# pdegenhardt/MinCostFlow

Hardware: AMD Instinct MI355X
Metric: pivots/sec + solve ms, NETGEN 100k-node/300k-arc; arc-scan GB/s vs HBM peak (higher is better)
Workload: dtype int64

## Files before the change

include/mcf_hip.h:

```cpp
#ifndef MCF_HIP_H
#define MCF_HIP_H

#include <stdint.h>

#ifdef __cplusplus
extern "C" {
#endif

#define MCF_API __attribute__((visibility("default")))

typedef enum mcf_status {
    MCF_OK = 0,
    MCF_ERR_INVALID = -1,
    MCF_ERR_NO_DEVICE = -2,
    MCF_ERR_HIP = -3,
    MCF_ERR_OVERFLOW = -4,
    MCF_ERR_TIMEOUT = -5,
    MCF_ERR_STATE = -6,
    MCF_ERR_IO = -7,
    MCF_ERR_COMM = -8
} mcf_status;

typedef enum mcf_pivot_rule { MCF_RULE_FIRST_ELIGIBLE = 0, MCF_RULE_BEST_ELIGIBLE = 1, MCF_RULE_BLOCK_SEARCH = 2,
                              MCF_RULE_CANDIDATE_LIST = 3, MCF_RULE_ALTERING_LIST = 4 } mcf_pivot_rule;
// ... 135 lines not shown
    int64_t scan_launches;
    int64_t update_launches;
    int64_t inline_updates;
    int64_t potential_nodes;
    int64_t arcs_scanned;
    int64_t timed_scans;
    double timed_scan_ns;
    double host_wait_ns;
    double host_launch_ns;
    int32_t scan_workgroups, scan_threads;
    int64_t bytes_per_scan;
    int64_t resident;
    int64_t resident_launches;
    int64_t resident_requests;
    double resident_scan_ns;
    double resident_kernel_ns;
    int64_t candidates;
    int64_t host_decided;
    int64_t arcs_checked;
    int32_t initial_block_size, current_block_size;
    int32_t comm_ranks;
    int32_t reserved;
    int64_t async_refreshes;
    int64_t scan_bytes_read;
    int64_t rc_layout;
    int64_t rc_recomputes;
    int64_t renumberings;
    int64_t heap_compactions;
    int64_t rc_reloads_in_grid;
    int64_t shift_grid;
    int64_t shift_lists;
    int64_t mirror_uploads;
    double phase_shift_ns, phase_values_ns, phase_scan_ns;
} mcf_engine_stats;
MCF_API int mcf_engine_get_stats(mcf_engine *e, mcf_engine_stats *out);
MCF_API int mcf_engine_reset_stats(mcf_engine *e);

MCF_API int mcf_engine_bench_scan(mcf_engine *e, int32_t reps, int32_t cold, int64_t flush_bytes,
                                  double *avg_ns, double *min_ns);

MCF_API int mcf_engine_bench_update(mcf_engine *e, int32_t count, int32_t reps, double *avg_ns, double *min_ns, int64_t *bytes);

MCF_API int mcf_engine_bench_search(mcf_engine *e, int32_t reps, double *avg_ns, double *min_ns);

MCF_API int mcf_comm_unique_id(uint8_t id_out[128]);
MCF_API int mcf_engine_comm_init(mcf_engine *e, const uint8_t id[128], int32_t rank, int32_t world);
MCF_API int mcf_engine_find_entering_sharded(mcf_engine *e, int32_t *found, int32_t *arc, int64_t *reduced_cost);

typedef struct mcf_exchange mcf_exchange;
MCF_API int mcf_exchange_open(mcf_exchange **out, const char *name, int32_t rank, int32_t world);
MCF_API void mcf_exchange_close(mcf_exchange *x);
MCF_API int mcf_exchange_all_gather(mcf_exchange *x, const mcf_candidate *mine, mcf_candidate *all );


typedef struct mcf_ns mcf_ns;

MCF_API int mcf_ns_create(mcf_ns **out, int32_t node_count, int32_t arc_count, const int32_t *source, const int32_t *target);
MCF_API void mcf_ns_destroy(mcf_ns *s);
MCF_API int mcf_ns_set_arc_bounds(mcf_ns *s, int32_t arc, int64_t lower, int64_t upper);
MCF_API int mcf_ns_set_arc_cost(mcf_ns *s, int32_t arc, int64_t cost);
MCF_API int mcf_ns_set_node_supply(mcf_ns *s, int32_t node, int64_t supply);
MCF_API int mcf_ns_set_problem(mcf_ns *s, const int64_t *lower, const int64_t *upper, const int64_t *cost, const int64_t *supply);
MCF_API int mcf_ns_set_supply_type(mcf_ns *s, int32_t type);
MCF_API int mcf_ns_set_pivot_rule(mcf_ns *s, int32_t rule);
MCF_API int mcf_ns_set_list_pivot_rule(mcf_ns *s, int32_t rule);
MCF_API int mcf_ns_enable_optimized_pivot(mcf_ns *s, int32_t enable);
// ... 442 lines not shown
```

mincostflow_amd/_lib.py:

```python
from __future__ import annotations

import ctypes as C
import importlib.util
import os
import re
import sys
import warnings

import numpy as np

_HERE = os.path.dirname(os.path.abspath(__file__))
LIB_PATH = os.path.join(_HERE, "libmcf_hip.so")

RULE_FIRST_ELIGIBLE, RULE_BEST_ELIGIBLE, RULE_BLOCK_SEARCH, RULE_CANDIDATE_LIST, RULE_ALTERING_LIST = 0, 1, 2, 3, 4
COLLECT_FIRST_N, COLLECT_BLOCKS = 0, 1
SEM_PLAIN, SEM_OPTIMIZED = 1, 2
VECTOR_DEFAULT, VECTOR_NONE = 0, -1
SUPPLY_GEQ, SUPPLY_LEQ = 0, 1
NOT_SOLVED, OPTIMAL, INFEASIBLE, UNBOUNDED, UNBALANCED = 0, 1, 2, 3, 4
STATE_UPPER, STATE_TREE, STATE_LOWER = -1, 0, 1
INF_CAP = np.iinfo(np.int64).max
ENGINE_SAMPLE_KERNEL_TIME, ENGINE_TIME_EVERY_KERNEL, ENGINE_NO_INLINE_UPDATE, ENGINE_RESIDENT, ENGINE_DISPATCH, ENGINE_CANDIDATES = 1, 2, 4, 8, 16, 32
ENGINE_SHARE_DEVICE = 64
ENGINE_NO_CANDIDATES = 128
ERR_INVALID, ERR_NO_DEVICE, ERR_HIP, ERR_OVERFLOW, ERR_TIMEOUT, ERR_STATE, ERR_IO, ERR_COMM = -1, -2, -3, -4, -5, -6, -7, -8


class McfError(RuntimeError):
    def __init__(self, code: int, message: str):
        super().__init__(f"mcf_hip error {code}: {message}")
        self.code = code


class EngineDesc(C.Structure):
    _fields_ = [(n, C.c_int32) for n in ("node_count", "arc_capacity", "search_arc_num", "int_width", "rule", "semantics",
                                         "block_size", "device", "shard_begin", "shard_end", "scan_workgroups", "flags", "resident_workgroups", "vector_width")]


class Candidate(C.Structure):
    _fields_ = [("reduced_cost", C.c_int64), ("pos", C.c_uint32), ("arc", C.c_int32),
                ("range_cost", C.c_int64), ("range_pos", C.c_uint32), ("range_arc", C.c_int32)]

    def __init__(self, reduced_cost=0, pos=0xFFFFFFFF, arc=-1, range_cost=0, range_pos=0xFFFFFFFF, range_arc=-1):
        super().__init__(reduced_cost, pos, arc, range_cost, range_pos, range_arc)


class EngineStats(C.Structure):
    _fields_ = [("searches", C.c_int64), ("scan_launches", C.c_int64), ("update_launches", C.c_int64),
                ("inline_updates", C.c_int64), ("potential_nodes", C.c_int64), ("arcs_scanned", C.c_int64),
                ("timed_scans", C.c_int64), ("timed_scan_ns", C.c_double), ("host_wait_ns", C.c_double),
                ("host_launch_ns", C.c_double), ("scan_workgroups", C.c_int32), ("scan_threads", C.c_int32),
                ("bytes_per_scan", C.c_int64), ("resident", C.c_int64), ("resident_launches", C.c_int64),
                ("resident_requests", C.c_int64), ("resident_scan_ns", C.c_double), ("resident_kernel_ns", C.c_double), ("candidates", C.c_int64),
                ("host_decided", C.c_int64), ("arcs_checked", C.c_int64), ("initial_block_size", C.c_int32), ("current_block_size", C.c_int32),
                ("comm_ranks", C.c_int32), ("reserved", C.c_int32), ("async_refreshes", C.c_int64), ("scan_bytes_read", C.c_int64), ("rc_layout", C.c_int64), ("rc_recomputes", C.c_int64), ("renumberings", C.c_int64), ("heap_compactions", C.c_int64), ("rc_reloads_in_grid", C.c_int64), ("shift_grid", C.c_int64), ("shift_lists", C.c_int64), ("mirror_uploads", C.c_int64),
                ("phase_shift_ns", C.c_double), ("phase_values_ns", C.c_double), ("phase_scan_ns", C.c_double)]

    def as_dict(self):
        return {n: getattr(self, n) for n, _ in self._fields_ if n != "reserved"}


OPT_NONE, OPT_ADAPTIVE_BLOCK_SIZE, OPT_SMALL_BLOCKS_FOR_DENSE, OPT_REDUCED_COST_CACHING = 0, 1, 2, 4


class BlockConfig(C.Structure):
    _fields_ = [("flags", C.c_int32), ("min_block_size", C.c_int32), ("max_block_size", C.c_int32), ("consecutive_hits_before_adapt", C.c_int32),
                ("min_block_size_ratio", C.c_double), ("block_size_growth_factor", C.c_double), ("block_size_shrink_factor", C.c_double),
                ("low_hit_rate_threshold", C.c_double), ("high_hit_rate_threshold", C.c_double)]

    def as_dict(self):
        return {n: getattr(self, n) for n, _ in self._fields_}


class NsMetrics(C.Structure):
    _fields_ = [("iterations", C.c_int64), ("total_solve_us", C.c_double), ("pivot_search_us", C.c_double),
                ("tree_update_us", C.c_double), ("potential_update_us", C.c_double), ("setup_us", C.c_double),
                ("loop_us", C.c_double), ("search_arc_num", C.c_int32),
                ("block_size", C.c_int32), ("int_width", C.c_int32), ("reserved", C.c_int32),
                ("degenerate_pivots", C.c_int64), ("potential_nodes", C.c_int64), ("engine", EngineStats),
                ("initial_block_size", C.c_int32), ("final_block_size", C.c_int32), ("total_arcs_checked", C.c_int64),
                ("average_arcs_checked_per_pivot", C.c_double), ("baseline_iterations", C.c_int32), ("config_flags", C.c_int32),
                ("iteration_ratio", C.c_double), ("reference_selects_cached_pivot", C.c_int32), ("reserved2", C.c_int32)]

    def as_dict(self):
        d = {n: getattr(self, n) for n, _ in self._fields_ if n not in ("engine", "reserved", "reserved2")}
        d["engine"] = self.engine.as_dict()
        return d


# ... 414 lines not shown
```

mincostflow_amd/csrc/candidate_cache.hip.h:

```cpp
#pragma once

constexpr int kCandMaxNodes = 256;
constexpr int kCandRefreshLow = 12;
constexpr int64_t kCandDegreePerNode = 8;
constexpr int kCandMaxAvgDegree = 24;

inline const int64_t *cand_pi(const mcf_engine *e) { return e->ext_pi ? e->ext_pi : e->pi.data(); }
inline bool cand_key_less(const mcf_engine::CandKey &a, const mcf_engine::CandKey &b) { return a.c < b.c || (a.c == b.c && a.p < b.p); }
struct CandHeapAfter {
    bool operator()(const mcf_engine::HeapEnt &a, const mcf_engine::HeapEnt &b) const { return b.c < a.c || (b.c == a.c && b.p < a.p); }
};

inline void cand_note_node(mcf_engine *e, int u, bool sigma_known = false, int64_t sigma = 0)
{
    if (e->rc_mode) {
        if (sigma_known) e->rc_sync.push_back(mcf_engine::NodeShift{u, sigma});
        else e->rc_shift_unknown = true;
    }
    if (e->blind_count > 0 && e->blind_epoch == e->cand_now) e->blind_sets = 2;
    if ((u == e->tp_u) | (u == e->tp_v)) e->tp_ok = false;
    if ((u == e->hd_u) | (u == e->hd_v)) e->hd_ok = false;
    if (e->node_at[u] != e->cand_now) {
        e->node_at[u] = e->cand_now;
        e->sync_nodes.push_back(u);
        if (!e->pivot_overflow) {
            e->pivot_nodes.push_back(u);
            e->pivot_degree += e->adj_start[u + 1] - e->adj_start[u];
            if ((int)e->pivot_nodes.size() > kCandMaxNodes || e->pivot_degree > kCandDegreePerNode * kCandMaxNodes) e->pivot_overflow = true;
        }
    }
}
inline void cand_note_arc(mcf_engine *e, int a)
{
    if (a == e->tp_a) e->tp_ok = false;
    if (a == e->hd_a) e->hd_ok = false;
    if (e->arc_at[a] != e->cand_now) { e->arc_at[a] = e->cand_now; e->sync_arcs.push_back(a); e->pivot_arcs.push_back(a); }
}
constexpr int kShiftRunMax = 256;

inline void cand_materialise_blind(mcf_engine *e)
{
    if (!e->blind_lazy) return;
    e->blind_lazy = false;
    std::vector<int32_t> ids;
// ... 29 lines not shown
        e->blind_count += (size_t)total;
    }
    if (e->async_posted && cand_records_ready(e, 0)) { const int rc = cand_collect(e, e->async_at); if (rc) return rc; }
    shift_stream(e);
    return MCF_OK;
}

inline int cand_note_nodes_blind(mcf_engine *e, int32_t count, const int32_t *nodes, const int64_t *values, bool continuation)
{
    if (e->blind_lazy) {
        if (e->shift_streamed > 0) { const int rc = resident_stop(e); if (rc) return rc; }
        cand_materialise_blind(e);
    }
    e->pivot_overflow = true;
    if (e->blind_count == 0) { e->blind_epoch = e->cand_now; e->blind_sets = 0; }
    if (!continuation) {
        e->blind_sets += 1;
        if (e->blind_sets > 1 && e->stream_lines > 0) { const int rc = resident_stop(e); if (rc) return rc; }
    }
    e->pend_node.insert(e->pend_node.end(), nodes, nodes + count);
    if (values) e->pend_val.insert(e->pend_val.end(), values, values + count);
    else {
        const size_t at = e->pend_val.size();
        e->pend_val.resize(at + (size_t)count);
        if (!e->shift_grid) for (int i = 0; i < count; ++i) e->pend_val[at + i] = e->ext_pi[nodes[i]];
    }
    e->blind_count = e->pend_node.size();
    if (e->async_posted && cand_records_ready(e, 0)) { const int rc = cand_collect(e, e->async_at); if (rc) return rc; }
    if (e->shift_grid) shift_stream(e);
    else resident_stream(e);
    return MCF_OK;
}

inline bool cand_heap_current(const mcf_engine *e, const mcf_engine::HeapEnt &t)
{
    return ((int)(e->arc_at[t.p] <= t.at) & (int)(e->node_at[t.u] <= t.at) & (int)(e->node_at[t.v] <= t.at)) != 0;
}

inline void cand_push(mcf_engine *e, int a)
{
    const int st = e->h_state[a];
    if (st == 0) return;
    const int64_t *pi = cand_pi(e);
    const int32_t u = e->h_src[a], v = e->h_tgt[a];
    const int64_t d = e->h_cost[a] + pi[u] - pi[v];
    const int64_t rc = st > 0 ? d : -d;
    if (rc >= 0) return;
    e->heap.push_back(mcf_engine::HeapEnt{rc, (uint32_t)a, e->cand_now, u, v});
    std::push_heap(e->heap.begin(), e->heap.end(), CandHeapAfter());
}

void cand_absorb_pivot(mcf_engine *e)
{
    if (e->pivot_overflow) {
        e->heap_gap = e->cand_now;
    } else {
        const int64_t *pi = cand_pi(e);
        const uint32_t now = e->cand_now;
        for (int u : e->pivot_nodes)
            for (int i = e->adj_start[u], hi = e->adj_start[u + 1]; i < hi; ++i) {
                const mcf_engine::AdjEnt &x = e->adj[i];
                __builtin_prefetch(&pi[x.other & 0x1FFFFFFFu]);
            }
        for (int u : e->pivot_nodes) {
            const int64_t pu = pi[u];
            for (int i = e->adj_start[u], hi = e->adj_start[u + 1]; i < hi; ++i) {
                const mcf_engine::AdjEnt &x = e->adj[i];
                const int st = (int)((x.other >> 29) & 3u) - 1;
                if (st == 0) continue;
                const int32_t other = (int32_t)(x.other & 0x1FFFFFFFu);
                const int64_t po = pi[other];
                const int64_t d = (x.other >> 31) ? x.cost + po - pu : x.cost + pu - po;
                const int64_t rc = st > 0 ? d : -d;
                if (rc >= 0) continue;
                e->heap.push_back(mcf_engine::HeapEnt{rc, (uint32_t)x.arc, now, u, other});
                std::push_heap(e->heap.begin(), e->heap.end(), CandHeapAfter());
            }
        }
        for (int a : e->pivot_arcs) cand_push(e, a);
    }
    e->pivot_nodes.clear();
    e->pivot_arcs.clear();
    e->pivot_degree = 0;
    e->pivot_overflow = false;
    if (e->heap.size() > e->heap_compact_above) {
        size_t keep = 0;
        for (size_t i = 0; i < e->heap.size(); ++i)
            if (cand_heap_current(e, e->heap[i])) e->heap[keep++] = e->heap[i];
        e->heap.resize(keep);
        std::make_heap(e->heap.begin(), e->heap.end(), CandHeapAfter());
        e->st.heap_compactions += 1;
    }
}

bool cand_decide(mcf_engine *e, Key *k)
{
    if (!e->cand_valid || e->snap_at < e->heap_gap) return false;
    mcf_engine::CandKey best_d{0, kNone};
    while (!e->heap.empty()) {
        const mcf_engine::HeapEnt &t = e->heap.front();
        const uint32_t a = t.p;
        if (e->tp_ok && (int32_t)a == e->tp_a && t.at == e->tp_at) { best_d = mcf_engine::CandKey{t.c, a}; break; }
        const bool after = t.at > e->snap_at;
        if (after && cand_heap_current(e, t)) {
            e->tp_ok = true; e->tp_a = (int32_t)a; e->tp_at = t.at; e->tp_u = t.u; e->tp_v = t.v;
            best_d = mcf_engine::CandKey{t.c, a};
            break;
        }
        std::pop_heap(e->heap.begin(), e->heap.end(), CandHeapAfter());
        e->heap.pop_back();
    }
    while (e->cand_ptr < e->cand_list.size()) {
        if (e->hd_ok && e->hd_ptr == e->cand_ptr) break;
        const uint32_t a = e->cand_list[e->cand_ptr].p;
        if (e->cand_ptr + 1 < e->cand_list.size()) {
            __builtin_prefetch(&e->arc_at[e->cand_list[e->cand_ptr + 1].p]);
            __builtin_prefetch(&e->node_at[e->cand_ends[2 * e->cand_ptr + 2]]);
            __builtin_prefetch(&e->node_at[e->cand_ends[2 * e->cand_ptr + 3]]);
        }
        const uint32_t t_arc = e->arc_at[a], t_src = e->node_at[e->cand_ends[2 * e->cand_ptr]], t_tgt = e->node_at[e->cand_ends[2 * e->cand_ptr + 1]];
        if ((t_arc <= e->snap_at) & (t_src <= e->snap_at) & (t_tgt <= e->snap_at)) {
            e->hd_ok = true; e->hd_ptr = e->cand_ptr; e->hd_a = (int32_t)a; e->hd_u = e->cand_ends[2 * e->cand_ptr]; e->hd_v = e->cand_ends[2 * e->cand_ptr + 1];
            break;
        }
        e->cand_ptr++;
    }
    mcf_engine::CandKey win{0, kNone};
    if (e->cand_ptr < e->cand_list.size()) {
        win = e->cand_list[e->cand_ptr];
        if (best_d.p != kNone && cand_key_less(best_d, win)) win = best_d;
    } else if (e->cand_thr.p == kNone) {
        win = best_d;
    } else if (best_d.p != kNone && cand_key_less(best_d, e->cand_thr)) {
        win = best_d;
    } else {
        return false;
    }
    k->c = win.p == kNone ? 0 : win.c;
    k->r = 0;
    k->p = win.p;
    return true;
}

int cand_build_patches(mcf_engine *e)
{
    const int64_t *pi = cand_pi(e);
    const size_t n_b = e->blind_count, n_s = e->sync_nodes.size();
    const bool blind_current = n_b == 0 || (e->blind_epoch == e->cand_now && e->blind_sets <= 1);
    const bool squeeze = (int64_t)n_b + (int64_t)n_s > e->patch_capacity;
    if ((!blind_current || squeeze) && e->stream_lines > 0) { const int rc = resident_stop(e); if (rc) return rc; }
    if (squeeze) {
        e->pend_node.insert(e->pend_node.end(), e->sync_nodes.begin(), e->sync_nodes.end());
        std::sort(e->pend_node.begin(), e->pend_node.end());
        e->pend_node.erase(std::unique(e->pend_node.begin(), e->pend_node.end()), e->pend_node.end());
        e->pend_val.resize(e->pend_node.size());
        for (size_t i = 0; i < e->pend_node.size(); ++i) e->pend_val[i] = pi[e->pend_node[i]];
    } else {
        if (!blind_current) for (size_t i = 0; i < n_b; ++i) e->pend_val[i] = pi[e->pend_node[i]];
        e->pend_node.resize(n_b + n_s);
        e->pend_val.resize(n_b + n_s);
        for (size_t i = 0; i < n_s; ++i) { e->pend_node[n_b + i] = e->sync_nodes[i]; e->pend_val[n_b + i] = pi[e->sync_nodes[i]]; }
    }
    e->pend_arc.assign(e->sync_arcs.begin(), e->sync_arcs.end());
    e->pend_state.resize(e->pend_arc.size());
    for (size_t i = 0; i < e->pend_arc.size(); ++i) e->pend_state[i] = e->h_state[e->pend_arc[i]];
    e->sync_nodes.clear();
    e->sync_arcs.clear();
    blind_clear(e);
    e->rc_sync.clear();
    e->rc_shift_unknown = false;
// ... 29 lines not shown
                int rc = resident_restart(e);
                if (rc) return rc;
            }
            if ((++spins & 0xFFFFF) == 0) {
                const hipError_t q = hipStreamQuery(e->res_stream ? e->res_stream : e->stream);
                if (q != hipSuccess && q != hipErrorNotReady) return mcf::fail(MCF_ERR_HIP, "resident grid failed: %s", hipGetErrorString(q));
                if (t0_wall == 0) t0_wall = mcf::now_ns();
                else if (mcf::now_ns() - t0_wall > 20e9) return mcf::fail(MCF_ERR_TIMEOUT, "no answer from the device after 20 s (workgroup %d of %d)", g, e->res_grid);
            }
        }
        std::atomic_thread_fence(std::memory_order_acquire);
        for (int r = 0; r < kCandPerGroup; ++r)
            if (rec[r].p != kNone) e->cand_list.push_back(mcf_engine::CandKey{rec[r].c, rec[r].p});
        if (rec[kCandPerGroup].p != kNone) {
            const mcf_engine::CandKey t{rec[kCandPerGroup].c, rec[kCandPerGroup].p};
            if (e->cand_thr.p == kNone || cand_key_less(t, e->cand_thr)) e->cand_thr = t;
        }
    }
    e->wait_ticks += (double)__rdtsc() - t0;
    if (e->cand_thr.p != kNone) {
        size_t keep = 0;
        for (size_t i = 0; i < e->cand_list.size(); ++i)
            if (cand_key_less(e->cand_list[i], e->cand_thr)) e->cand_list[keep++] = e->cand_list[i];
        e->cand_list.resize(keep);
    }
    std::sort(e->cand_list.begin(), e->cand_list.end(), cand_key_less);
    e->cand_ends.resize(2 * e->cand_list.size());
    for (size_t i = 0; i < e->cand_list.size(); ++i) { e->cand_ends[2 * i] = e->h_src[e->cand_list[i].p]; e->cand_ends[2 * i + 1] = e->h_tgt[e->cand_list[i].p]; }
    e->cand_ptr = 0;
    e->cand_valid = true;
    e->hd_ok = e->tp_ok = false;
    e->snap_at = at;
    e->async_posted = false;
    e->tk_collect += (double)__rdtsc() - t0;
    return MCF_OK;
}

int cand_post_rc(mcf_engine *e)
{
    const bool reload = e->reload_pi && e->d_ext_pi != nullptr && (int64_t)e->sync_arcs.size() <= e->mailbox_max_st;
    if (reload) {
        pend_clear_potentials(e);
        e->sync_nodes.clear(); e->rc_sync.clear(); e->rc_shift_unknown = false;
        blind_clear(e);
        e->reload_pi = false;
    }
    const size_t n_b = e->blind_count, n_s = e->rc_sync.size();
    const bool blind_ok = n_b == 0 || (e->pend_shift && e->blind_epoch == e->cand_now);
    const int64_t n_st = (int64_t)e->sync_arcs.size();
    const bool fast = !e->reload_pi && !e->rc_shift_unknown && blind_ok && (int64_t)(n_b + n_s) <= (int64_t)e->rc_list_max && n_st <= e->mailbox_max_st;
    if (fast) {
        e->pend_node.resize(n_b + n_s);
        e->pend_val.resize(n_b + n_s);
        for (size_t i = 0; i < n_b; ++i) e->pend_val[i] = e->pend_sigma;
        for (size_t i = 0; i < n_s; ++i) { e->pend_node[n_b + i] = e->rc_sync[i].node; e->pend_val[n_b + i] = e->rc_sync[i].shift; }
        e->pend_arc.assign(e->sync_arcs.begin(), e->sync_arcs.end());
        e->pend_state.resize(e->pend_arc.size());
        for (size_t i = 0; i < e->pend_arc.size(); ++i) e->pend_state[i] = e->h_state[e->pend_arc[i]];
        e->sync_nodes.clear(); e->sync_arcs.clear(); e->rc_sync.clear();
        blind_clear(e);
    } else {
        if (int rcb = cand_build_patches(e)) return rcb;
        int rc = resident_stop(e);
        if (!rc) rc = flush_pending(e);
        if (rc) return rc;
    }
// ... 172 lines not shown
    e->posted_at = e->cand_now;
    e->st.arcs_scanned += e->end - e->begin;
    return MCF_OK;
}

void cand_build_adjacency(mcf_engine *e)
{
    const int n = e->d.node_count, m_s = e->d.search_arc_num;
    const int32_t *source = e->h_src.data(), *target = e->h_tgt.data();
    const int lo = e->begin, hi = std::min(e->end, m_s);
    e->adj_start.assign(n + 1, 0);
    for (int a = lo; a < hi; ++a) { e->adj_start[source[a] + 1]++; if (target[a] != source[a]) e->adj_start[target[a] + 1]++; }
    for (int u = 0; u < n; ++u) e->adj_start[u + 1] += e->adj_start[u];
    e->adj.assign(e->adj_start[n], mcf_engine::AdjEnt{0, 0u, 0});
    e->adj_pos.assign((size_t)2 * m_s, -1);
    std::vector<int32_t> fill(e->adj_start.begin(), e->adj_start.end() - 1);
    for (int a = lo; a < hi; ++a) {
        const uint32_t st_bits = (uint32_t)(e->h_state[a] + 1) << 29;
        e->adj_pos[2 * (size_t)a] = fill[source[a]];
        e->adj[fill[source[a]]++] = mcf_engine::AdjEnt{a, (uint32_t)target[a] | st_bits, e->h_cost[a]};
        if (target[a] != source[a]) {
            e->adj_pos[2 * (size_t)a + 1] = fill[target[a]];
            e->adj[fill[target[a]]++] = mcf_engine::AdjEnt{a, (uint32_t)source[a] | st_bits | 0x80000000u, e->h_cost[a]};
        }
    }
}

void cand_reset(mcf_engine *e)
{
    e->cand_valid = false;
    e->cand_list.clear();
    e->cand_ptr = 0;
    e->hd_ok = e->tp_ok = false;
    e->heap.clear();
    e->pivot_nodes.clear(); e->pivot_arcs.clear(); e->pivot_degree = 0; e->pivot_overflow = false;
    e->heap_gap = e->cand_now;
}
```

mincostflow_amd/csrc/engine.hip:

```cpp
#include <hip/hip_runtime.h>
#include <hip/hip_ext.h>
#include <hsa/hsa.h>
#include <hsa/hsa_ext_amd.h>

#include <dlfcn.h>
#include <immintrin.h>

#include <algorithm>
#include <atomic>
#include <cmath>
#include <cstdio>
#include <cstring>
#include <map>
#include <mutex>
#include <vector>

#include "common.h"

#include "kernels.hip.h"
#include "collect.hip.h"

namespace {

#define HIP_TRY(expr)                                                                                      \
    do {                                                                                                   \
        hipError_t err__ = (expr);                                                                         \
        if (err__ != hipSuccess) return mcf::fail(MCF_ERR_HIP, "%s: %s", #expr, hipGetErrorString(err__)); \
    } while (0)

struct Id128 { char b[128]; };
typedef int (*nccl_get_unique_id_t)(Id128 *);
typedef int (*nccl_comm_init_rank_t)(void **, int, Id128, int);
typedef int (*nccl_all_gather_t)(const void *, void *, size_t, int, void *, hipStream_t);
typedef int (*nccl_comm_destroy_t)(void *);
typedef const char *(*nccl_get_error_string_t)(int);
typedef int (*nccl_comm_count_t)(void *, int *);
struct RcclApi {
    void *lib = nullptr;
    nccl_get_unique_id_t get_unique_id = nullptr;
    nccl_comm_init_rank_t comm_init_rank = nullptr;
    nccl_all_gather_t all_gather = nullptr;
    nccl_comm_destroy_t comm_destroy = nullptr;
    nccl_get_error_string_t error_string = nullptr;
    nccl_comm_count_t comm_count = nullptr;
};
RcclApi *rccl()
{
    static RcclApi api;
    static std::once_flag once;
    std::call_once(once, [] {
// ... 89 lines not shown
    bool comm_resident = false;
    bool resident_ok = false, resident_running = false, resident_reg = false;
    bool has_slot = false;
    int shift_reload_min = 0;
    bool shift_grid = false;
    uint32_t shift_base = 0;
    int max_shift_lines = 0;
    int cand_tiles = 1;
    int shift_streamed = 0;
    double wait_ticks = 0, launch_ticks = 0, cal_ns = 0, cal_ticks = 0;
    enum { kNoSearch = 0, kAnswered, kResidentSearch, kCandSearch, kDispatchSearch } in_flight = kNoSearch;
    Key answered{0, kNone, kNone};
    Key range_key{0, kNone, kNone};
    int vec = 0;
    bool in_flight_timed = false;
    int stream_lines = 0;
    uint32_t stream_sub = 0;
    uint32_t *mailbox = nullptr;
    int mailbox_lines = 0, mailbox_max_st = 0;
    uint32_t idle_ticks = 0;
    uint32_t prev_seq = 0;
    bool cand_on = false, cand_valid = false;
    mcf::hvec<int32_t> h_src, h_tgt;
    mcf::hvec<int64_t> h_cost;
    mcf::hvec<int8_t> h_state;
    struct AdjEnt { int32_t arc; uint32_t other; int64_t cost; };
    mcf::hvec<int32_t> adj_start;
    mcf::hvec<AdjEnt> adj;
    mcf::hvec<uint32_t> node_at, arc_at;
    mcf::hvec<int32_t> adj_pos;
    uint32_t cand_now = 1;
    uint32_t snap_at = 0;
    uint32_t heap_gap = 0;
    struct CandKey { int64_t c; uint32_t p; };
    struct HeapEnt { int64_t c; uint32_t p; uint32_t at; int32_t u, v; };
    std::vector<HeapEnt> heap;
    std::vector<int32_t> pivot_nodes, pivot_arcs;
    int64_t pivot_degree = 0;
    bool pivot_overflow = false;
    std::vector<int32_t> sync_nodes, sync_arcs;
    size_t blind_count = 0;
    std::vector<uint32_t> blind_runs;
    bool blind_lazy = false;
    uint32_t blind_epoch = 0;
    int blind_sets = 0;
    bool force_device_search = false;
    bool cand_appending = false;
    struct NodeShift { int32_t node; int64_t shift; };
    std::vector<NodeShift> rc_sync;
    bool rc_shift_unknown = false;
    bool call_shift_known = false;
    int64_t call_shift = 0;
    std::vector<CandKey> cand_list;
    std::vector<int32_t> cand_ends;
    size_t cand_ptr = 0;
    bool tp_ok = false, hd_ok = false;
    int32_t tp_a = -1, tp_u = -1, tp_v = -1, hd_a = -1, hd_u = -1, hd_v = -1;
    uint32_t tp_at = 0;
    size_t hd_ptr = 0;
    CandKey cand_thr{0, 0xFFFFFFFFu};
    bool async_posted = false;
    uint32_t async_at = 0, posted_at = 0;
    int patch_capacity = 0;
    uint32_t cand_epoch0 = 1;
    size_t heap_compact_above = 1u << 18;
    bool cand_debug = false;
    double tk_absorb = 0, tk_decide = 0, tk_post = 0, tk_collect = 0, tk_probe = 0;
    int64_t n_sync_posts = 0, n_async_waits = 0, n_gap_pivots = 0, n_heap_push = 0, n_heap_pop = 0, n_list_skip = 0;
    uint32_t *h_exit = nullptr, *d_exit = nullptr;
    int res_grid = 0, res_threads = kResidentThreads;
    hipEvent_t res_start = nullptr, res_stop = nullptr;
    void *d_flush = nullptr;
    size_t flush_bytes = 0;
    bool list_rule = false;
    std::vector<int32_t> pend_index;
    CollectTile *d_tiles = nullptr;
    CollectHeader *h_collect_hdr = nullptr, *d_collect_hdr = nullptr;
    CollectEntry *h_collect = nullptr, *d_collect = nullptr;
    int collect_cap = 0;
};

namespace {
inline void blind_clear(mcf_engine *e)
{
    e->blind_count = 0;
    e->blind_runs.clear();
    e->blind_lazy = false;
}

#include "engine_helpers.hip.h"

bool fits32(int64_t v) { return v >= INT32_MIN && v <= INT32_MAX; }

int drain_events(mcf_engine *e, bool all)
{
    while (e->ev_tail != e->ev_head) {
        const int i = e->ev_tail % mcf_engine::kEvRing;
        if (!all && hipEventQuery(e->ev_stop[i]) != hipSuccess) break;
// ... 619 lines not shown
                                desc->node_count <= kShiftBits;
                if (e->shift_grid) {
                    const int64_t groups4 = ((int64_t)count + kArcsPerThread - 1) / kArcsPerThread;
                    e->cand_tiles = groups4 <= (int64_t)2 * e->res_grid * kCandThreads ? 2 : 4;
                    const int64_t t = std::max<int64_t>(64, ((groups4 + (int64_t)e->cand_tiles * e->res_grid - 1) / ((int64_t)e->cand_tiles * e->res_grid) + 63) / 64 * 64);
                    if (t > kCandThreads) e->shift_grid = false;
                    else e->res_threads = (int)t;
                }
                if (e->shift_grid) {
                    e->shift_reload_min = (int)mcf::env_int("MCF_HIP_SHIFT_RELOAD", 0, INT32_MAX, 32768);
                    if (e->shift_reload_min > 0 && hipMalloc((void **)&e->d_barrier, 64) != hipSuccess) { e->d_barrier = nullptr; (void)hipGetLastError(); }
                }
            }
        }
    }
    e->st.scan_workgroups = e->resident_ok ? e->res_grid : e->grid;
    {
        int want = (count >= kBucketMinArcs && desc->node_count > 2 * kBucketNodes) ? kBucketNodes : 0;
        want = (int)mcf::env_int("MCF_HIP_BUCKET_NODES", 0, INT32_MAX, want);
        const bool tile_loop = !e->lds_pi && !(e->resident_ok && e->resident_reg) && !e->rc_mode;
        if (want > 0 && desc->rule == MCF_RULE_BEST_ELIGIBLE && tile_loop && !e->cand_on) {
            if (hipMalloc((void **)&e->d_orig, sizeof(int32_t) * e->count_padded) == hipSuccess) e->bucket_nodes = want;
        }
    }
    e->st.scan_threads = e->resident_ok ? e->res_threads : (e->lds_pi ? kResidentThreads : kThreads);
    e->st.resident = e->resident_ok ? 1 : 0;
    e->st.candidates = e->cand_on ? 1 : 0;
    e->st.bytes_per_scan = (int64_t)(desc->int_width == 64 ? 17 : 13) * count + (int64_t)w * desc->node_count;
    e->st.scan_bytes_read = e->rc_mode ? (int64_t)9 * count : e->st.bytes_per_scan;
    e->st.rc_layout = e->rc_mode ? 1 : 0;
    e->st.shift_grid = e->shift_grid ? 1 : 0;
    e->st.initial_block_size = e->st.current_block_size = e->block_size;
    e->cand_epoch0 = (uint32_t)mcf::env_int("MCF_HIP_CAND_EPOCH0", 1, 0xFFFFFFFFll, 1);
    e->heap_compact_above = (size_t)mcf::env_int("MCF_HIP_CAND_HEAP_COMPACT", 1, 1ll << 30, (long long)e->heap_compact_above);
    e->cand_debug = getenv("MCF_HIP_CAND_DEBUG") != nullptr;
    *out = e;
    return MCF_OK;
}

namespace {
std::mutex g_pin_mutex;
std::map<const void *, int> g_pins;
bool host_pin(const void *p, size_t bytes)
{
    std::lock_guard<std::mutex> lock(g_pin_mutex);
    auto it = g_pins.find(p);
    if (it != g_pins.end()) { it->second += 1; return true; }
    const hipError_t r = hipHostRegister(const_cast<void *>(p), bytes, hipHostRegisterPortable | hipHostRegisterMapped);
    (void)hipGetLastError();
    if (r != hipSuccess) return false;
    g_pins[p] = 1;
    return true;
}
void host_unpin(const void *p)
{
    std::lock_guard<std::mutex> lock(g_pin_mutex);
    auto it = g_pins.find(p);
    if (it == g_pins.end()) return;
    if (--it->second > 0) return;
    g_pins.erase(it);
    (void)hipHostUnregister(const_cast<void *>(p));
    (void)hipGetLastError();
}
}

void mcf_engine_destroy(mcf_engine *e)
{
    if (!e) return;
    if (e->cand_on && e->cand_debug && e->st.searches > 1000) {
        const double ns_per_tick = (mcf::now_ns() - e->cal_ns) / std::max(1.0, (double)__rdtsc() - e->cal_ticks);
        const double n = (double)e->st.searches;
        fprintf(stderr, "[cand] searches %lld host %lld async %lld sync_posts %lld async_waits %lld gap_pivots %lld | per search ns: absorb %.0f probe %.0f decide %.0f post %.0f collect %.0f wait %.0f | heap size %zu\n",
                (long long)e->st.searches, (long long)e->st.host_decided, (long long)e->st.async_refreshes, (long long)e->n_sync_posts, (long long)e->n_async_waits,
                (long long)e->n_gap_pivots, e->tk_absorb * ns_per_tick / n, e->tk_probe * ns_per_tick / n, e->tk_decide * ns_per_tick / n, e->tk_post * ns_per_tick / n,
                e->tk_collect * ns_per_tick / n, e->wait_ticks * ns_per_tick / n, e->heap.size());
    }
    (void)hipSetDevice(e->d.device);
    (void)resident_stop(e);
    if (e->ext_pi && e->ext_pi_pinned) { if (e->stream) (void)hipStreamSynchronize(e->stream); host_unpin(e->ext_pi); }
    if (e->stream) (void)hipStreamSynchronize(e->stream);
    if (e->res_stream) { (void)hipStreamSynchronize(e->res_stream); (void)hipStreamDestroy(e->res_stream); e->res_stream = nullptr; }
    if (e->mailbox) hsa_amd_memory_pool_free(e->mailbox);
    if (e->h_exit) (void)hipHostFree(e->h_exit);
    if (e->res_start) (void)hipEventDestroy(e->res_start);
    if (e->res_stop) (void)hipEventDestroy(e->res_stop);
    if (e->comm && rccl() && rccl()->comm_destroy) rccl()->comm_destroy(e->comm);
    if (e->d_orig) (void)hipFree(e->d_orig);
    (void)hipFree(e->d_rc); (void)hipFree(e->d_adj_start); (void)hipFree(e->d_adj); (void)hipFree(e->d_barrier); (void)hipFree(e->d_node_map);
    (void)hipFree(e->d_src); (void)hipFree(e->d_tgt); (void)hipFree(e->d_cost); (void)hipFree(e->d_state); (void)hipFree(e->d_pi);
    (void)hipFree(e->d_cand_local); (void)hipFree(e->d_cand_all); (void)hipFree(e->d_flush); (void)hipFree(e->d_dev_slots);
    (void)hipFree(e->d_tiles);
    if (e->h_collect_hdr) (void)hipHostFree(e->h_collect_hdr);
    if (e->h_collect) (void)hipHostFree(e->h_collect);
    if (e->h_cand_all) (void)hipHostFree(e->h_cand_all);
    if (e->comm_stream) { (void)hipStreamSynchronize(e->comm_stream); (void)hipStreamDestroy(e->comm_stream); }
    if (e->x_send) (void)hipHostFree(e->x_send);
    if (e->x_recv) (void)hipHostFree(e->x_recv);
    if (e->h_slots) (void)hipHostFree(e->h_slots);
    for (auto &s : e->stage) {
        if (s.nodes) (void)hipHostFree(s.nodes);
        if (s.values) (void)hipHostFree(s.values);
        if (s.arcs) (void)hipHostFree(s.arcs);
        if (s.states) (void)hipHostFree(s.states);
        if (s.done) (void)hipEventDestroy(s.done);
    }
    for (int i = 0; i < mcf_engine::kEvRing; ++i) {
        if (e->ev_start[i]) (void)hipEventDestroy(e->ev_start[i]);
        if (e->ev_stop[i]) (void)hipEventDestroy(e->ev_stop[i]);
// ... 507 lines not shown
    hipError_t err = hipMemcpyAsync(e->d_node_map, new_of, sizeof(int32_t) * (size_t)n, hipMemcpyHostToDevice, e->stream);
    if (err == hipSuccess) {
        hipLaunchKernelGGL(renumber_kernel, dim3(e->count_padded / kThreads), dim3(kThreads), 0, e->stream, e->d_src, e->d_tgt, e->d_node_map, e->count_padded);
        err = hipGetLastError();
    }
    if (err == hipSuccess) err = hipStreamSynchronize(e->stream);
    if (err != hipSuccess) return mcf::fail(MCF_ERR_HIP, "mcf_engine_renumber_nodes: %s", hipGetErrorString(err));
    if (!e->ext_pi) {
        if (!e->mirror_valid) { rc = mcf_engine_download_pi(e, e->pi.data()); if (rc) return rc; e->mirror_valid = true; }
        mcf::hvec<int64_t> moved((size_t)n);
        for (int u = 0; u < n; ++u) moved[new_of[u]] = e->pi[u];
        std::copy(moved.begin(), moved.end(), e->pi.begin());
    }
    {
        const int64_t *pi = e->ext_pi ? e->ext_pi : e->pi.data();
        if (e->d.int_width == 32) {
            std::vector<int32_t> p32((size_t)n);
            for (int u = 0; u < n; ++u) { if (!fits32(pi[u])) return mcf::fail(MCF_ERR_OVERFLOW, "potential of node %d does not fit int32", u); p32[u] = (int32_t)pi[u]; }
            HIP_TRY(hipMemcpyAsync(e->d_pi, p32.data(), sizeof(int32_t) * (size_t)n, hipMemcpyHostToDevice, e->stream));
            HIP_TRY(hipStreamSynchronize(e->stream));
        } else {
            HIP_TRY(hipMemcpyAsync(e->d_pi, pi, sizeof(int64_t) * (size_t)n, hipMemcpyHostToDevice, e->stream));
            HIP_TRY(hipStreamSynchronize(e->stream));
        }
    }
    if (e->cand_on) {
        const int m_s = e->d.search_arc_num;
        for (int a = 0; a < m_s; ++a) { e->h_src[a] = new_of[e->h_src[a]]; e->h_tgt[a] = new_of[e->h_tgt[a]]; }
        cand_build_adjacency(e);
        mcf::hvec<uint32_t> at((size_t)n);
        for (int u = 0; u < n; ++u) at[new_of[u]] = e->node_at[u];
        std::copy(at.begin(), at.end(), e->node_at.begin());
        for (size_t i = 0; i < e->cand_ends.size(); ++i) e->cand_ends[i] = new_of[e->cand_ends[i]];
        for (auto &h : e->heap) { h.u = new_of[h.u]; h.v = new_of[h.v]; }
        e->tp_ok = e->hd_ok = false;
        for (int32_t &u : e->pivot_nodes) u = new_of[u];
        for (int32_t &u : e->sync_nodes) u = new_of[u];
        for (auto &x : e->rc_sync) x.node = new_of[x.node];
    }
    if (e->rc_mode) {
        const int cnt = e->end - e->begin;
        std::vector<int32_t> s2((size_t)std::max(1, cnt)), t2((size_t)std::max(1, cnt));
        if (e->cand_on) { std::copy(e->h_src.begin() + e->begin, e->h_src.begin() + e->end, s2.begin()); std::copy(e->h_tgt.begin() + e->begin, e->h_tgt.begin() + e->end, t2.begin()); }
        else {
            HIP_TRY(hipMemcpy(s2.data(), e->d_src, sizeof(int32_t) * cnt, hipMemcpyDeviceToHost));
            HIP_TRY(hipMemcpy(t2.data(), e->d_tgt, sizeof(int32_t) * cnt, hipMemcpyDeviceToHost));
        }
        rc = rc_build_adjacency(e, s2.data(), t2.data());
        if (!rc) rc = rc_recompute(e);
        if (rc) return rc;
        HIP_TRY(hipStreamSynchronize(e->stream));
    }
    e->st.renumberings += 1;
    return MCF_OK;
}

int mcf_engine_find_entering(mcf_engine *e, int32_t *found, int32_t *arc, int64_t *reduced_cost)
{
    if (!e || !found || !arc) return mcf::fail(MCF_ERR_INVALID, "mcf_engine_find_entering: null argument");
    if (e->begin != 0 || e->end != e->d.search_arc_num) return mcf::fail(MCF_ERR_STATE, "sharded engine: use mcf_engine_find_entering_local / _sharded");
    Key k;
    int rc = local_search(e, &k);
    if (rc) return rc;
    resolve_key(e, k, found, arc, reduced_cost);
    return MCF_OK;
}

// ... 206 lines not shown
    }
    return MCF_OK;
}

int mcf_engine_download_state(mcf_engine *e, int8_t *out)
{
    if (!e || !out) return mcf::fail(MCF_ERR_INVALID, "null argument");
    HIP_TRY(hipSetDevice(e->d.device));
    int rc = resident_stop(e);
    if (!rc) rc = flush_pending(e);
    if (rc) return rc;
    HIP_TRY(hipStreamSynchronize(e->stream));
    if (e->bucket_nodes > 0) {
        std::vector<int8_t> stored(e->end - e->begin);
        HIP_TRY(hipMemcpy(stored.data(), e->d_state, stored.size(), hipMemcpyDeviceToHost));
        for (int i = 0; i < e->end - e->begin; ++i) out[e->begin + i] = stored[e->pos_of[i]];
        return MCF_OK;
    }
    HIP_TRY(hipMemcpy(out + e->begin, e->d_state, e->end - e->begin, hipMemcpyDeviceToHost));
    return MCF_OK;
}

int mcf_engine_get_stats(mcf_engine *e, mcf_engine_stats *out)
{
    if (!e || !out) return mcf::fail(MCF_ERR_INVALID, "null argument");
    (void)hipSetDevice(e->d.device);
    int rc = resident_stop(e);
    if (!rc) rc = drain_events(e, true);
    if (rc) return rc;
    const double ns_per_tick = (mcf::now_ns() - e->cal_ns) / std::max(1.0, (double)__rdtsc() - e->cal_ticks);
    e->st.host_wait_ns = e->wait_ticks * ns_per_tick;
    e->st.host_launch_ns = e->launch_ticks * ns_per_tick;
    e->st.current_block_size = e->block_size;
    *out = e->st;
    return MCF_OK;
}

int mcf_engine_reset_stats(mcf_engine *e)
{
    if (!e) return mcf::fail(MCF_ERR_INVALID, "null argument");
    (void)hipSetDevice(e->d.device);
    drain_events(e, true);
    const mcf_engine_stats keep = e->st;
    e->st = mcf_engine_stats{};
    e->wait_ticks = e->launch_ticks = 0;
    e->st.scan_workgroups = keep.scan_workgroups;
    e->st.scan_threads = keep.scan_threads;
    e->st.bytes_per_scan = keep.bytes_per_scan;
    e->st.resident = keep.resident;
    e->st.candidates = keep.candidates;
    e->st.initial_block_size = keep.initial_block_size;
    e->st.current_block_size = e->block_size;
    e->st.comm_ranks = keep.comm_ranks;
    e->st.scan_bytes_read = keep.scan_bytes_read;
    e->st.rc_layout = keep.rc_layout;
    e->st.shift_grid = keep.shift_grid;
    return MCF_OK;
}

int mcf_engine_bench_scan(mcf_engine *e, int32_t reps, int32_t cold, int64_t flush_bytes, double *avg_ns, double *min_ns)
{
    if (!e || reps < 1 || !avg_ns || !min_ns) return mcf::fail(MCF_ERR_INVALID, "mcf_engine_bench_scan: bad arguments");
    if (e->list_rule) return mcf::fail(MCF_ERR_STATE, "engines of the list rules (3, 4) are searched with mcf_engine_collect_eligible only");
    if (!e->uploaded) return mcf::fail(MCF_ERR_STATE, "mcf_engine_upload has not been called");
    HIP_TRY(hipSetDevice(e->d.device));
    int rc = resident_stop(e);
    if (!rc) rc = flush_pending(e);
    if (rc) return rc;
    if (cold) {
        const size_t want = (size_t)std::max<int64_t>(flush_bytes, 1 << 20);
        if (e->flush_bytes < want) {
            (void)hipFree(e->d_flush);
            e->d_flush = nullptr;
            HIP_TRY(hipMalloc(&e->d_flush, want));
            HIP_TRY(hipMemset(e->d_flush, 0, want));
            e->flush_bytes = want;
        }
    }
// ... 231 lines not shown
```

Baseline: 254,100.

## Defer touched candidates at or above threshold instead of pushing them onto heap

Replaces the host-side candidate heap with a TouchedKeys structure. Entries whose reduced cost does not beat the current candidate-list threshold go to an unordered deferred vector instead of the binary heap. On each new snapshot install, stale heap entries are pruned and still-fresh deferred entries below the new threshold are readmitted. This is meant to cut push_heap/pop_heap cost and heap growth during host-decided pivots, at the price of extra install-time filtering and more bookkeeping. New stats counters are also exposed.

```diff
diff --git a/include/mcf_hip.h b/include/mcf_hip.h
--- a/include/mcf_hip.h
+++ b/include/mcf_hip.h
@@ -191,6 +191,10 @@
     int64_t shift_lists;
     int64_t mirror_uploads;
     double phase_shift_ns, phase_values_ns, phase_scan_ns;
+    int64_t cand_admitted;
+    int64_t cand_deferred;
+    int64_t cand_readmitted;
+    int64_t cand_heap_max;
 } mcf_engine_stats;
 MCF_API int mcf_engine_get_stats(mcf_engine *e, mcf_engine_stats *out);
 MCF_API int mcf_engine_reset_stats(mcf_engine *e);
diff --git a/mincostflow_amd/_lib.py b/mincostflow_amd/_lib.py
--- a/mincostflow_amd/_lib.py
+++ b/mincostflow_amd/_lib.py
@@ -54,7 +54,8 @@
                 ("resident_requests", C.c_int64), ("resident_scan_ns", C.c_double), ("resident_kernel_ns", C.c_double), ("candidates", C.c_int64),
                 ("host_decided", C.c_int64), ("arcs_checked", C.c_int64), ("initial_block_size", C.c_int32), ("current_block_size", C.c_int32),
                 ("comm_ranks", C.c_int32), ("reserved", C.c_int32), ("async_refreshes", C.c_int64), ("scan_bytes_read", C.c_int64), ("rc_layout", C.c_int64), ("rc_recomputes", C.c_int64), ("renumberings", C.c_int64), ("heap_compactions", C.c_int64), ("rc_reloads_in_grid", C.c_int64), ("shift_grid", C.c_int64), ("shift_lists", C.c_int64), ("mirror_uploads", C.c_int64),
-                ("phase_shift_ns", C.c_double), ("phase_values_ns", C.c_double), ("phase_scan_ns", C.c_double)]
+                ("phase_shift_ns", C.c_double), ("phase_values_ns", C.c_double), ("phase_scan_ns", C.c_double),
+                ("cand_admitted", C.c_int64), ("cand_deferred", C.c_int64), ("cand_readmitted", C.c_int64), ("cand_heap_max", C.c_int64)]
 
     def as_dict(self):
         return {n: getattr(self, n) for n, _ in self._fields_ if n != "reserved"}
diff --git a/mincostflow_amd/csrc/candidate_cache.hip.h b/mincostflow_amd/csrc/candidate_cache.hip.h
--- a/mincostflow_amd/csrc/candidate_cache.hip.h
+++ b/mincostflow_amd/csrc/candidate_cache.hip.h
@@ -6,10 +6,7 @@
 constexpr int kCandMaxAvgDegree = 24;
 
 inline const int64_t *cand_pi(const mcf_engine *e) { return e->ext_pi ? e->ext_pi : e->pi.data(); }
-inline bool cand_key_less(const mcf_engine::CandKey &a, const mcf_engine::CandKey &b) { return a.c < b.c || (a.c == b.c && a.p < b.p); }
-struct CandHeapAfter {
-    bool operator()(const mcf_engine::HeapEnt &a, const mcf_engine::HeapEnt &b) const { return b.c < a.c || (b.c == a.c && b.p < a.p); }
-};
+inline bool cand_key_less(const mcf_engine::CandKey &a, const mcf_engine::CandKey &b) { return mcf::touched_key_less(a, b); }
 
 inline void cand_note_node(mcf_engine *e, int u, bool sigma_known = false, int64_t sigma = 0)
 {
@@ -105,11 +102,6 @@
     return MCF_OK;
 }
 
-inline bool cand_heap_current(const mcf_engine *e, const mcf_engine::HeapEnt &t)
-{
-    return ((int)(e->arc_at[t.p] <= t.at) & (int)(e->node_at[t.u] <= t.at) & (int)(e->node_at[t.v] <= t.at)) != 0;
-}
-
 inline void cand_push(mcf_engine *e, int a)
 {
     const int st = e->h_state[a];
@@ -119,8 +111,7 @@
     const int64_t d = e->h_cost[a] + pi[u] - pi[v];
     const int64_t rc = st > 0 ? d : -d;
     if (rc >= 0) return;
-    e->heap.push_back(mcf_engine::HeapEnt{rc, (uint32_t)a, e->cand_now, u, v});
-    std::push_heap(e->heap.begin(), e->heap.end(), CandHeapAfter());
+    e->touched.push(mcf::TouchedEnt{rc, (uint32_t)a, e->cand_now, u, v}, e->cand_thr);
 }
 
 void cand_absorb_pivot(mcf_engine *e)
@@ -130,6 +121,7 @@
     } else {
         const int64_t *pi = cand_pi(e);
         const uint32_t now = e->cand_now;
+        const mcf_engine::CandKey thr = e->cand_thr;
         for (int u : e->pivot_nodes)
             for (int i = e->adj_start[u], hi = e->adj_start[u + 1]; i < hi; ++i) {
                 const mcf_engine::AdjEnt &x = e->adj[i];
@@ -146,8 +138,7 @@
                 const int64_t d = (x.other >> 31) ? x.cost + po - pu : x.cost + pu - po;
                 const int64_t rc = st > 0 ? d : -d;
                 if (rc >= 0) continue;
-                e->heap.push_back(mcf_engine::HeapEnt{rc, (uint32_t)x.arc, now, u, other});
-                std::push_heap(e->heap.begin(), e->heap.end(), CandHeapAfter());
+                e->touched.push(mcf::TouchedEnt{rc, (uint32_t)x.arc, now, u, other}, thr);
             }
         }
         for (int a : e->pivot_arcs) cand_push(e, a);
@@ -156,33 +147,15 @@
     e->pivot_arcs.clear();
     e->pivot_degree = 0;
     e->pivot_overflow = false;
-    if (e->heap.size() > e->heap_compact_above) {
-        size_t keep = 0;
-        for (size_t i = 0; i < e->heap.size(); ++i)
-            if (cand_heap_current(e, e->heap[i])) e->heap[keep++] = e->heap[i];
-        e->heap.resize(keep);
-        std::make_heap(e->heap.begin(), e->heap.end(), CandHeapAfter());
-        e->st.heap_compactions += 1;
-    }
+    if (e->touched.sweep(e->node_at.data(), e->arc_at.data(), e->snap_at, e->async_posted, e->async_at)) e->st.heap_compactions += 1;
 }
 
 bool cand_decide(mcf_engine *e, Key *k)
 {
     if (!e->cand_valid || e->snap_at < e->heap_gap) return false;
-    mcf_engine::CandKey best_d{0, kNone};
-    while (!e->heap.empty()) {
-        const mcf_engine::HeapEnt &t = e->heap.front();
-        const uint32_t a = t.p;
-        if (e->tp_ok && (int32_t)a == e->tp_a && t.at == e->tp_at) { best_d = mcf_engine::CandKey{t.c, a}; break; }
-        const bool after = t.at > e->snap_at;
-        if (after && cand_heap_current(e, t)) {
-            e->tp_ok = true; e->tp_a = (int32_t)a; e->tp_at = t.at; e->tp_u = t.u; e->tp_v = t.v;
-            best_d = mcf_engine::CandKey{t.c, a};
-            break;
-        }
-        std::pop_heap(e->heap.begin(), e->heap.end(), CandHeapAfter());
-        e->heap.pop_back();
-    }
+    bool looked_up = false;
+    const mcf::TouchedEnt *const best = e->touched.top(e->node_at.data(), e->arc_at.data(), e->snap_at, e->tp_ok, (uint32_t)e->tp_a, e->tp_at, &looked_up);
+    if (looked_up) { e->tp_ok = true; e->tp_a = (int32_t)best->p; e->tp_at = best->at; e->tp_u = best->u; e->tp_v = best->v; }
     while (e->cand_ptr < e->cand_list.size()) {
         if (e->hd_ok && e->hd_ptr == e->cand_ptr) break;
         const uint32_t a = e->cand_list[e->cand_ptr].p;
@@ -198,17 +171,8 @@
         }
         e->cand_ptr++;
     }
-    mcf_engine::CandKey win{0, kNone};
-    if (e->cand_ptr < e->cand_list.size()) {
-        win = e->cand_list[e->cand_ptr];
-        if (best_d.p != kNone && cand_key_less(best_d, win)) win = best_d;
-    } else if (e->cand_thr.p == kNone) {
-        win = best_d;
-    } else if (best_d.p != kNone && cand_key_less(best_d, e->cand_thr)) {
-        win = best_d;
-    } else {
-        return false;
-    }
+    mcf_engine::CandKey win;
+    if (!mcf::TouchedKeys::winner(e->cand_ptr < e->cand_list.size() ? &e->cand_list[e->cand_ptr] : nullptr, e->cand_thr, best, &win)) return false;
     k->c = win.p == kNone ? 0 : win.c;
     k->r = 0;
     k->p = win.p;
@@ -304,6 +268,7 @@
     e->hd_ok = e->tp_ok = false;
     e->snap_at = at;
     e->async_posted = false;
+    e->touched.install(at, e->cand_thr);
     e->tk_collect += (double)__rdtsc() - t0;
     return MCF_OK;
 }
@@ -542,7 +507,7 @@
     e->cand_list.clear();
     e->cand_ptr = 0;
     e->hd_ok = e->tp_ok = false;
-    e->heap.clear();
+    e->touched.clear();
     e->pivot_nodes.clear(); e->pivot_arcs.clear(); e->pivot_degree = 0; e->pivot_overflow = false;
     e->heap_gap = e->cand_now;
 }
diff --git a/mincostflow_amd/csrc/engine.hip b/mincostflow_amd/csrc/engine.hip
--- a/mincostflow_amd/csrc/engine.hip
+++ b/mincostflow_amd/csrc/engine.hip
@@ -16,6 +16,7 @@
 #include <vector>
 
 #include "common.h"
+#include "touched_keys.h"
 
 #include "kernels.hip.h"
 #include "collect.hip.h"
@@ -171,9 +172,8 @@
     uint32_t cand_now = 1;
     uint32_t snap_at = 0;
     uint32_t heap_gap = 0;
-    struct CandKey { int64_t c; uint32_t p; };
-    struct HeapEnt { int64_t c; uint32_t p; uint32_t at; int32_t u, v; };
-    std::vector<HeapEnt> heap;
+    using CandKey = mcf::TouchedKey;
+    mcf::TouchedKeys touched;
     std::vector<int32_t> pivot_nodes, pivot_arcs;
     int64_t pivot_degree = 0;
     bool pivot_overflow = false;
@@ -202,7 +202,6 @@
     uint32_t async_at = 0, posted_at = 0;
     int patch_capacity = 0;
     uint32_t cand_epoch0 = 1;
-    size_t heap_compact_above = 1u << 18;
     bool cand_debug = false;
     double tk_absorb = 0, tk_decide = 0, tk_post = 0, tk_collect = 0, tk_probe = 0;
     int64_t n_sync_posts = 0, n_async_waits = 0, n_gap_pivots = 0, n_heap_push = 0, n_heap_pop = 0, n_list_skip = 0;
@@ -888,7 +887,7 @@
     e->st.shift_grid = e->shift_grid ? 1 : 0;
     e->st.initial_block_size = e->st.current_block_size = e->block_size;
     e->cand_epoch0 = (uint32_t)mcf::env_int("MCF_HIP_CAND_EPOCH0", 1, 0xFFFFFFFFll, 1);
-    e->heap_compact_above = (size_t)mcf::env_int("MCF_HIP_CAND_HEAP_COMPACT", 1, 1ll << 30, (long long)e->heap_compact_above);
+    e->touched.bound = (size_t)mcf::env_int("MCF_HIP_CAND_HEAP_COMPACT", 1, 1ll << 30, (long long)e->touched.bound);
     e->cand_debug = getenv("MCF_HIP_CAND_DEBUG") != nullptr;
     *out = e;
     return MCF_OK;
@@ -926,10 +925,11 @@
     if (e->cand_on && e->cand_debug && e->st.searches > 1000) {
         const double ns_per_tick = (mcf::now_ns() - e->cal_ns) / std::max(1.0, (double)__rdtsc() - e->cal_ticks);
         const double n = (double)e->st.searches;
-        fprintf(stderr, "[cand] searches %lld host %lld async %lld sync_posts %lld async_waits %lld gap_pivots %lld | per search ns: absorb %.0f probe %.0f decide %.0f post %.0f collect %.0f wait %.0f | heap size %zu\n",
+        fprintf(stderr, "[cand] searches %lld host %lld async %lld sync_posts %lld async_waits %lld gap_pivots %lld | per search ns: absorb %.0f probe %.0f decide %.0f post %.0f collect %.0f wait %.0f | heap size %zu max %zu | entries admitted %lld deferred %lld re-admitted %lld\n",
                 (long long)e->st.searches, (long long)e->st.host_decided, (long long)e->st.async_refreshes, (long long)e->n_sync_posts, (long long)e->n_async_waits,
                 (long long)e->n_gap_pivots, e->tk_absorb * ns_per_tick / n, e->tk_probe * ns_per_tick / n, e->tk_decide * ns_per_tick / n, e->tk_post * ns_per_tick / n,
-                e->tk_collect * ns_per_tick / n, e->wait_ticks * ns_per_tick / n, e->heap.size());
+                e->tk_collect * ns_per_tick / n, e->wait_ticks * ns_per_tick / n, e->touched.heap.size(), e->touched.heap_max,
+                (long long)e->touched.admitted, (long long)e->touched.deferrals, (long long)e->touched.readmitted);
     }
     (void)hipSetDevice(e->d.device);
     (void)resident_stop(e);
@@ -1503,7 +1503,8 @@
         for (int u = 0; u < n; ++u) at[new_of[u]] = e->node_at[u];
         std::copy(at.begin(), at.end(), e->node_at.begin());
         for (size_t i = 0; i < e->cand_ends.size(); ++i) e->cand_ends[i] = new_of[e->cand_ends[i]];
-        for (auto &h : e->heap) { h.u = new_of[h.u]; h.v = new_of[h.v]; }
+        for (auto &h : e->touched.heap) { h.u = new_of[h.u]; h.v = new_of[h.v]; }
+        for (auto &h : e->touched.deferred) { h.u = new_of[h.u]; h.v = new_of[h.v]; }
         e->tp_ok = e->hd_ok = false;
         for (int32_t &u : e->pivot_nodes) u = new_of[u];
         for (int32_t &u : e->sync_nodes) u = new_of[u];
@@ -1776,6 +1777,10 @@
     e->st.host_wait_ns = e->wait_ticks * ns_per_tick;
     e->st.host_launch_ns = e->launch_ticks * ns_per_tick;
     e->st.current_block_size = e->block_size;
+    e->st.cand_admitted = e->touched.admitted;
+    e->st.cand_deferred = e->touched.deferrals;
+    e->st.cand_readmitted = e->touched.readmitted;
+    e->st.cand_heap_max = (int64_t)e->touched.heap_max;
     *out = e->st;
     return MCF_OK;
 }
@@ -1788,6 +1793,8 @@
     const mcf_engine_stats keep = e->st;
     e->st = mcf_engine_stats{};
     e->wait_ticks = e->launch_ticks = 0;
+    e->touched.admitted = e->touched.deferrals = e->touched.readmitted = 0;
+    e->touched.heap_max = e->touched.heap.size();
     e->st.scan_workgroups = keep.scan_workgroups;
     e->st.scan_threads = keep.scan_threads;
     e->st.bytes_per_scan = keep.bytes_per_scan;
diff --git a/mincostflow_amd/csrc/touched_keys.h b/mincostflow_amd/csrc/touched_keys.h
--- /dev/null
+++ b/mincostflow_amd/csrc/touched_keys.h
@@ -0,0 +1,112 @@
+#pragma once
+
+#include <stddef.h>
+#include <stdint.h>
+
+#include <algorithm>
+#include <vector>
+
+namespace mcf {
+
+constexpr uint32_t kNoTouchedArc = 0xFFFFFFFFu;
+
+struct TouchedKey { int64_t c; uint32_t p; };
+inline bool touched_key_less(const TouchedKey &a, const TouchedKey &b) { return a.c < b.c || (a.c == b.c && a.p < b.p); }
+
+struct TouchedEnt { int64_t c; uint32_t p; uint32_t at; int32_t u, v; };
+
+struct TouchedKeys {
+    struct After {
+        bool operator()(const TouchedEnt &a, const TouchedEnt &b) const { return b.c < a.c || (b.c == a.c && b.p < a.p); }
+    };
+    std::vector<TouchedEnt> heap;
+    std::vector<TouchedEnt> deferred;
+    size_t bound = 1u << 18;
+    int64_t admitted = 0, deferrals = 0, readmitted = 0, sweeps = 0;
+    size_t heap_max = 0;
+
+    void clear() { heap.clear(); deferred.clear(); }
+    size_t size() const { return heap.size() + deferred.size(); }
+
+    static bool current(const uint32_t *node_at, const uint32_t *arc_at, const TouchedEnt &t)
+    {
+        return ((int)(arc_at[t.p] <= t.at) & (int)(node_at[t.u] <= t.at) & (int)(node_at[t.v] <= t.at)) != 0;
+    }
+
+    void push(const TouchedEnt &t, const TouchedKey &thr)
+    {
+        if (thr.p != kNoTouchedArc && !touched_key_less(TouchedKey{t.c, t.p}, thr)) {
+            deferred.push_back(t);
+            deferrals += 1;
+            return;
+        }
+        heap.push_back(t);
+        std::push_heap(heap.begin(), heap.end(), After());
+        admitted += 1;
+        if (heap.size() > heap_max) heap_max = heap.size();
+    }
+
+    const TouchedEnt *top(const uint32_t *node_at, const uint32_t *arc_at, uint32_t snap_at, bool known, uint32_t known_p, uint32_t known_at, bool *looked_up)
+    {
+        *looked_up = false;
+        while (!heap.empty()) {
+            const TouchedEnt &t = heap.front();
+            if (known && t.p == known_p && t.at == known_at) return &t;
+            if (t.at > snap_at && current(node_at, arc_at, t)) { *looked_up = true; return &t; }
+            std::pop_heap(heap.begin(), heap.end(), After());
+            heap.pop_back();
+        }
+        return nullptr;
+    }
+
+    void install(uint32_t at, const TouchedKey &thr)
+    {
+        const bool all = thr.p == kNoTouchedArc;
+        size_t keep = 0;
+        for (size_t i = 0; i < heap.size(); ++i)
+            if (heap[i].at > at && (all || touched_key_less(TouchedKey{heap[i].c, heap[i].p}, thr))) heap[keep++] = heap[i];
+        heap.resize(keep);
+        size_t lo = deferred.size();
+        while (lo > 0 && deferred[lo - 1].at > at) --lo;
+        for (size_t i = lo; i < deferred.size(); ++i)
+            if (all || touched_key_less(TouchedKey{deferred[i].c, deferred[i].p}, thr)) { heap.push_back(deferred[i]); readmitted += 1; }
+        deferred.clear();
+        std::make_heap(heap.begin(), heap.end(), After());
+        if (heap.size() > heap_max) heap_max = heap.size();
+    }
+
+    bool sweep(const uint32_t *node_at, const uint32_t *arc_at, uint32_t snap_at, bool pending, uint32_t pending_at)
+    {
+        if (size() <= bound) return false;
+        size_t keep = 0;
+        for (size_t i = 0; i < heap.size(); ++i)
+            if (heap[i].at > snap_at && current(node_at, arc_at, heap[i])) heap[keep++] = heap[i];
+        heap.resize(keep);
+        std::make_heap(heap.begin(), heap.end(), After());
+        keep = 0;
+        if (pending)
+            for (size_t i = 0; i < deferred.size(); ++i)
+                if (deferred[i].at > pending_at && current(node_at, arc_at, deferred[i])) deferred[keep++] = deferred[i];
+        deferred.resize(keep);
+        sweeps += 1;
+        return true;
+    }
+
+    static bool winner(const TouchedKey *listed, const TouchedKey &thr, const TouchedEnt *best, TouchedKey *win)
+    {
+        *win = TouchedKey{0, kNoTouchedArc};
+        if (listed) {
+            *win = *listed;
+            if (best && touched_key_less(TouchedKey{best->c, best->p}, *win)) *win = TouchedKey{best->c, best->p};
+        } else if (thr.p == kNoTouchedArc) {
+            if (best) *win = TouchedKey{best->c, best->p};
+        } else if (best && touched_key_less(TouchedKey{best->c, best->p}, thr)) {
+            *win = TouchedKey{best->c, best->p};
+        } else {
+            return false;
+        }
+        return true;
+    }
+};
+
+}
```

After: 287,300 (median of 5 runs). +13.1%, better.
